# yweweler/single-speaker-tts

Measured on AMD Instinct MI355X. Metric: mel-frames/sec (end-to-end text->waveform incl. 60-iter Griffin-Lim, 64-utt LJ-Speech-shaped batch per GPU), higher is better.
Workload: dtype f32

## Files before the change

### single-speaker-tts_amd/csrc/gl_plan.h

```cpp
#pragma once
#include <cstddef>
#include <vector>

namespace tts {

constexpr int NFFT = 2048;
constexpr int MH = NFFT / 2;
constexpr int GL_NW = 8;
constexpr int EX_CPLX = 1088;
constexpr int CT_SWORDS = 16;
constexpr int GL_LDS_BUDGET = 160 * 1024;

struct GlItem { int b, t0, len, slot; };

struct GlStreamGeom { int wpad, halo, lag, S, acc_len; };
GlStreamGeom gl_stream_geom(int win, int hop);

int gl_stream_ring_frames(int win, int hop, int n_stage = 1);
size_t gl_stream_lds_bytes(int win, int hop, int ring_frames, int n_stage);

inline int gl_rw_edge_len(int n_fft, int win, int hop) { return n_fft + ((win + hop - 1) / hop - 1) * hop; }

void gl_build_wlane(const float* window, const float* rwss, int win, int hop, int T, float* out);

int gl_plan_items(const int* lens, int T, int B, int win, int hop, int n_workers, int n_stage, int force_runs, int force_run_len,
                  std::vector<GlItem>* items, int* slots_per_utt, int* workers_out = nullptr);

}
```

### single-speaker-tts_amd/csrc/gl_plan.hip

```cpp
#include "gl_plan.h"
#include <algorithm>
#include <cmath>
#include <utility>

namespace tts {

GlStreamGeom gl_stream_geom(int win, int hop) {
    GlStreamGeom g;
    g.wpad = (NFFT - win) >> 1;
    g.halo = (win + hop - 1) / hop - 1;
    g.lag = (g.halo + 1) * hop > 2 * (MH - g.wpad) ? g.halo : g.halo + 1;
    const int c_lo = g.wpad >> 7, c_hi = (g.wpad + win - 1) >> 7;
    g.S = 128 * (c_hi - c_lo + 1);
    g.acc_len = g.S - hop;
    return g;
}

static constexpr size_t GL_LDS_FIXED = (size_t)GL_NW * EX_CPLX * 2 * sizeof(float) + CT_SWORDS * sizeof(int);

int gl_stream_ring_frames(int win, int hop, int n_stage) {
    const GlStreamGeom g = gl_stream_geom(win, hop);
    if (g.acc_len < 0) return 0;
    const int budget = (GL_LDS_BUDGET - (int)GL_LDS_FIXED) / (int)sizeof(float) / n_stage - g.acc_len - 132;
    int need = 9 + g.lag + (g.S + hop - 1) / hop + 1;
    const int reach = (g.S + win + 2 * hop + hop - 1) / hop;
    need = std::max(need, std::max(reach, GL_NW));
    const int R = std::min(budget / hop, std::max(64, need));
    return R >= need ? R : 0;
}

size_t gl_stream_lds_bytes(int win, int hop, int ring_frames, int n_stage) {
    const GlStreamGeom g = gl_stream_geom(win, hop);
    return GL_LDS_FIXED + (size_t)(n_stage < 1 ? 1 : n_stage) * (size_t)((hop * ring_frames + g.acc_len + 128 + 3) & ~3) * sizeof(float);
}

void gl_build_wlane(const float* window, const float* rwss, int win, int hop, int T, float* out) {
    const GlStreamGeom g = gl_stream_geom(win, hop);
    const int t_ref = g.halo < T ? g.halo : T - 1;
    for (int c = 0; c < 16; ++c)
        for (int e = 0; e < 2; ++e)
            for (int lane = 0; lane < 64; ++lane) {
                const int nw = 2 * (lane + 64 * c) + e - g.wpad;
                const bool in = nw >= 0 && nw < win;
                const float w = in ? window[nw] * (0.5f / (float)MH) : 0.f;
                const float rw = in ? rwss[(size_t)t_ref * hop + g.wpad + nw] : 0.f;
                out[(0 * 64 + lane) * 32 + 2 * c + e] = w;
                out[(1 * 64 + lane) * 32 + 2 * c + e] = w * rw;
            }
}

namespace {
struct GlRun { int b, t0, len, ord = 0; };
struct GlCutCost { double interior, edge; };
GlCutCost gl_cut_cost(int halo, int lag, int n_stage) {
    const double c = (halo + lag) * n_stage / 4.0;
    return GlCutCost{c * (5.5 / 6.0), c * 0.5};
}
template <bool STORE>
bool gl_deal(const int* lens, int T, int B, int W, double M, const GlCutCost& cc, int min_len_all, std::vector<std::vector<GlRun>>& workers, double* makespan,
             double give_up = 1e300) {
    if (STORE) workers.assign((size_t)W, {});
    bool w_empty = true;
    int b = 0, t = 0, w = 0;
    double load = 0.0, worst = 0.0;
    while (b < B) {
        if (w >= W) return false;
        const int Tb = lens ? lens[b] : T;
        const int min_len = std::min(Tb, min_len_all);
        const int rest = Tb - t;
        const double left = t > 0 ? cc.interior : cc.edge;
        const double whole = rest + left + cc.edge;
        if (load + whole <= M + 1e-9) {
            if (STORE) workers[w].push_back(GlRun{b, t, rest});
            w_empty = false;
            load += whole;
            ++b; t = 0;
            continue;
        }
        int len = (int)std::floor(M - load - left - cc.interior + 1e-9);
        if (rest - len < min_len) len = rest - min_len;
        if (len >= min_len) {
            if (STORE) workers[w].push_back(GlRun{b, t, len});
            load += len + left + cc.interior;
            t += len;
        } else if (w_empty) {
            return false;
        }
        worst = std::max(worst, load);
        if (!STORE && worst >= give_up) return false;
        ++w; load = 0.0; w_empty = true;
    }
    worst = std::max(worst, load);
    if (makespan) *makespan = worst;
    return true;
}
}

int gl_plan_items(const int* lens, int T, int B, int win, int hop, int n_workers, int n_stage, int force_runs, int force_run_len,
                  std::vector<GlItem>* items, int* slots_per_utt, int* workers_out) {
    auto len_of = [&](int b) { return lens ? lens[b] : T; };
    long long total_frames = 0;
    int T_min = len_of(0), T_top = len_of(0);
    for (int b = 0; b < B; ++b) {
        total_frames += len_of(b);
        T_min = std::min(T_min, len_of(b));
        T_top = std::max(T_top, len_of(b));
    }
    if (lens && T_min == T_top) {
        lens = nullptr;
        T = T_top;
    }
    const GlStreamGeom g = gl_stream_geom(win, hop);
    n_stage = n_stage < 1 ? 1 : (n_stage > 3 ? 3 : n_stage);
    n_workers = n_workers < 1 ? 1 : n_workers;
    std::vector<std::vector<GlRun>> workers;
    int forced_len = 0;
    if (force_runs >= 1 && force_runs <= T_top) forced_len = ((T_top + force_runs - 1) / force_runs + GL_NW - 1) / GL_NW * GL_NW;
    if (force_run_len >= GL_NW) forced_len = force_run_len / GL_NW * GL_NW;
    if (forced_len > 0) {
        for (int t0 = 0; t0 < T_top; t0 += forced_len)
            for (int b = 0; b < B; ++b)
                if (t0 < len_of(b)) workers.push_back({GlRun{b, t0, std::min(forced_len, len_of(b) - t0)}});
    } else {
        const GlCutCost cc = gl_cut_cost(g.halo, g.lag, n_stage);
        const long long per_worker = total_frames / n_workers;
        const int min_len_all = (int)std::max<long long>(GL_NW / 2, std::min<long long>(GL_NW, per_worker));
        const int min_len = std::min(T_min, min_len_all);
        const double total = (double)total_frames + (double)B * 2 * cc.edge;
        double lo = std::max(total / n_workers, (double)min_len + 2 * cc.edge), best_t = 1e300;
        std::vector<std::vector<GlRun>> none;
        int best_step = -1;
        double best_M = 0.0;
        for (int step = 0; step < 400; ++step) {
            const double M = lo * (1.0 + 0.0025 * step);
            double t = 0.0;
            if (!gl_deal<false>(lens, T, B, n_workers, M, cc, min_len_all, none, &t, best_t - 1e-9)) continue;
            if (t < best_t - 1e-9) { best_t = t; best_M = M; best_step = step; }
        }
        if (lens && best_step > 0) {
            for (int sub = 1; sub < 16; ++sub) {
                const double M = lo * (1.0 + 0.0025 * (best_step - 1 + sub / 16.0));
                double t = 0.0;
                if (!gl_deal<false>(lens, T, B, n_workers, M, cc, min_len_all, none, &t, best_t - 1e-9)) continue;
                if (t < best_t - 1e-9) { best_t = t; best_M = M; }
            }
        }
        if (best_step >= 0) gl_deal<true>(lens, T, B, n_workers, best_M, cc, min_len_all, workers, nullptr);
        if (workers.empty()) {
            for (int b = 0; b < B; ++b) workers.push_back({GlRun{b, 0, len_of(b)}});
        }
    }
    std::vector<int> runs_of((size_t)B, 0);
    for (auto& w : workers) for (GlRun& r : w) r.ord = runs_of[r.b]++;
    int spu = 1;
    for (int b = 0; b < B; ++b) spu = std::max(spu, runs_of[b]);
    auto item_of = [&](const GlRun& r) {
        const int ord = r.ord;
        const int pad = ord == runs_of[r.b] - 1 ? spu - runs_of[r.b] : 0;
        return GlItem{r.b, r.t0, r.len, ord | (pad << 16)};
    };
    typedef std::pair<double, const GlRun*> Start;
    const auto earlier = [](const Start& a, const Start& b) { return a.first < b.first; };
    items->clear();
    size_t depth = 0;
    for (const auto& w : workers) depth = std::max(depth, w.size());
    if (lens) {
        std::vector<Start> rest;
        for (const auto& w : workers) {
            double before = 0.0;
            for (size_t d = 0; d < w.size(); ++d) {
                if (d == 0) items->push_back(item_of(w[d]));
                else rest.push_back({before, &w[d]});
                before += w[d].len + 11.0;
            }
        }
        std::stable_sort(rest.begin(), rest.end(), earlier);
        for (const auto& e : rest) items->push_back(item_of(*e.second));
        depth = 0;
    }
    for (size_t d = 0; d < depth; ++d) {
        std::vector<Start> level;
        for (const auto& w : workers) {
            if (w.size() <= d) continue;
            double before = 0.0;
            for (size_t q = 0; q < d; ++q) before += w[q].len;
            level.push_back({before, &w[d]});
// ... 15 lines not shown
```

### single-speaker-tts_amd/csrc/griffin_lim.hip

```cpp
#include "tts_common.h"
#include "griffin_lim.h"
#include "fft_wave.h"
#include <algorithm>
#include <cmath>
#include <cstdlib>

namespace tts {


__device__ __forceinline__ void lds_barrier() {
    asm volatile("s_waitcnt lgkmcnt(0)\n\ts_barrier" ::: "memory");
}

typedef __attribute__((address_space(3))) int gl_lds_int;
__device__ __forceinline__ int gl_flag_load(int* p) {
    return __hip_atomic_load((gl_lds_int*)p, __ATOMIC_RELAXED, __HIP_MEMORY_SCOPE_WORKGROUP);
}
__device__ __forceinline__ void gl_flag_store(int* p, int v) {
    __hip_atomic_store((gl_lds_int*)p, v, __ATOMIC_RELAXED, __HIP_MEMORY_SCOPE_WORKGROUP);
}

__device__ __forceinline__ void mirror_bins(const cf (&z)[16], cf (&m)[16], cf* ex, int lane, cf nyq) {
    cf* wr = ex + lane;
    const cf* rd = ex + (1024 - lane);
#pragma unroll
    for (int c = 0; c < 16; ++c) wr[64 * c] = z[c];
    if (lane == 0) ex[1024] = nyq;
    wave_lds_sync();
#pragma unroll
    for (int c = 0; c < 16; ++c) m[c] = rd[-64 * c];
    wave_lds_sync();
}

#define GL_BIN(lane, j) ((j) < 8 ? (lane) + 64 * (j) : MH - (lane) - 64 * ((j) - 8))
#define GL_ROW(LO, HI, j) ((j) < 8 ? (LO)[64 * (j)] : (HI)[-64 * ((j) - 8)])
#define GL_THREADS 512

__device__ __forceinline__ float gl_stream_load(const float* p) { return __builtin_nontemporal_load(p); }
__device__ __forceinline__ void gl_stream_store(cf* p, cf v) { __builtin_nontemporal_store(v, p); }
#define GL_STREAM_LOAD(ptr) gl_stream_load(ptr)
#define GL_STREAM_STORE(ptr, val) gl_stream_store((ptr), (val))
__device__ __forceinline__ cf gl_seed_phasor(unsigned long long seed, unsigned long long idx) {
    unsigned x = (unsigned)idx ^ ((unsigned)(idx >> 32) * 0x9E3779B9u) ^ (unsigned)seed ^ ((unsigned)(seed >> 32) * 0x85EBCA6Bu);
    x ^= x >> 16; x *= 0x7FEB352Du; x ^= x >> 15; x *= 0x846CA68Bu; x ^= x >> 16;
    const float u = (float)(x >> 8) * (1.0f / 16777216.0f);
    return cmk(__builtin_amdgcn_cosf(u), __builtin_amdgcn_sinf(u));
}
__device__ __forceinline__ unsigned gl_pack_phasor(cf x) {
    const float den = fmaxf(fabsf(x.x) + fabsf(x.y), 1.0e-30f);
    const float p = x.y * __builtin_amdgcn_rcpf(den);
    return (__float_as_uint(p) & ~1u) | (__float_as_uint(x.x) >> 31);
}
__device__ __forceinline__ cf gl_unpack_phasor(unsigned c, float mag) {
    const float p = __uint_as_float(c);
    const float q = 1.0f - fabsf(p);
    const float xs = __uint_as_float(__float_as_uint(q) | (c << 31));
    const float g = mag * __builtin_amdgcn_rsqf(fmaf(p, p, q * q));
    return cmk(xs, p) * g;
}

__device__ __forceinline__ cf gl_normalise(cf x, float mag) {
    const float xr = x.x + 1.0e-17f;
    const float s2 = fmaf(xr, xr, fmaf(x.y, x.y, 1.0e-38f));
    const float g = mag * __builtin_amdgcn_rsqf(s2);
    return cmk(xr, x.y) * g;
}
typedef unsigned gl_state_t;
__device__ __forceinline__ gl_state_t gl_state_encode(cf x) { return gl_pack_phasor(x); }
__device__ __forceinline__ cf gl_state_decode(gl_state_t s, float mag) { return gl_unpack_phasor(s, mag); }
size_t gl_state_bytes() { return sizeof(gl_state_t); }

#define GL_NO_ITEM 0x7FFFFFFEu
enum { CT_OLA = 0, CT_SNEXT = 1, CT_OLB = 2  };

template <int MODE, int WIN_CT, int HOP_CT, bool MSE, int NST = 1, bool SEEDED = false, bool MOM = false, bool RAG = false>
__global__ __launch_bounds__(GL_THREADS) void gl_stream_kernel(GlParams p) {
    static_assert(!SEEDED || MODE == 0, "the seeded start is an iteration's");
    static_assert(!MOM || (MODE == 0 && NST == 1), "momentum: one iteration per launch");
    static_assert(NST == 1 || (NST >= 2 && NST <= 3 && MODE == 0 && !MSE), "several iterations per launch: plain iterations only");
    extern __shared__ __attribute__((aligned(16))) unsigned char smem_raw[];
    const int win = WIN_CT ? WIN_CT : p.win;
    const int hop = HOP_CT ? HOP_CT : p.hop;
    const int ncol = (WIN_CT && HOP_CT) ? (WIN_CT + HOP_CT - 1) / (HOP_CT ? HOP_CT : 1) : p.ncol;
    const int halo = ncol - 1;
    const int wpad = (NFFT - win) >> 1;
    const int c_lo = wpad >> 7;
    const int c_hi = (wpad + win - 1) >> 7;
    constexpr int fz_lo_ = WIN_CT ? ((NFFT - WIN_CT) >> 1) >> 7 : 0;
    constexpr int fz_hi_ = WIN_CT ? (((NFFT - WIN_CT) >> 1) + WIN_CT - 1) >> 7 : 15;
    constexpr bool fz_ok_ = fz_lo_ <= 4 && fz_hi_ >= 11 && fz_hi_ <= 15;
    constexpr int FZ_LO = fz_ok_ ? fz_lo_ : 0, FZ_HI = fz_ok_ ? fz_hi_ : 15;
    const int n_sl = c_hi - c_lo + 1;
    const int S = 128 * n_sl;
    const int fs = 128 * c_lo;
    const int acc_len = S - hop;
    const int lag = (halo + 1) * hop > 2 * (MH - wpad) ? halo : halo + 1;
    const int R = p.ring_frames;
    const int ring_len = hop * R;
    const int ring_floats = (ring_len + acc_len + 128 + 3) & ~3;
    const int L = hop * (p.T - 1);
    int Tb_r = p.T;
    int L_r = L;
    const float* rw_head = nullptr;
    const float* rw_tail = nullptr;
#define GL_TB (RAG ? Tb_r : p.T)
#define GL_L (RAG ? L_r : L)
    cf* ex_all = reinterpret_cast<cf*>(smem_raw);
    int* ctrl = reinterpret_cast<int*>(ex_all + GL_NW * EX_CPLX);
    float* ringA = reinterpret_cast<float*>(ctrl + CT_SWORDS);

    const int tid = threadIdx.x;
    const int lane = tid & 63;
    const int wave = __builtin_amdgcn_readfirstlane(tid >> 6);
    cf* ex = ex_all + wave * EX_CPLX;

    if (tid == 0) ctrl[CT_SNEXT] = (int)atomicAdd(p.work_counter, 1u);
    if (tid == 0 && blockIdx.x == 0 && p.clear_counter) *p.clear_counter = 0u;
    cf twr[8];
#pragma unroll
    for (int j = 0; j < 8; ++j) twr[j] = reinterpret_cast<const cf*>(p.tw2048)[lane + 64 * j];
    FftTwReg tw;
#pragma unroll
    for (int k2 = 1; k2 < 16; ++k2) tw.a[k2 - 1] = reinterpret_cast<const cf*>(p.tables)[1024 + (k2 - 1) * 64 + lane];
#pragma unroll
    for (int d = 1; d < 4; ++d) tw.b[d - 1] = reinterpret_cast<const cf*>(p.tw1024)[16 * (lane & 15) * d];
    float wana[16][2], wsyn[16][2];
    {
        const float4* wa = reinterpret_cast<const float4*>(p.wlane + (0 * 64 + lane) * 32);
        const float4* ws = reinterpret_cast<const float4*>(p.wlane + (1 * 64 + lane) * 32);
#pragma unroll
        for (int q = 0; q < 8; ++q) {
            const float4 a4 = wa[q], s4 = ws[q];
            wana[2 * q][0] = a4.x; wana[2 * q][1] = a4.y; wana[2 * q + 1][0] = a4.z; wana[2 * q + 1][1] = a4.w;
            wsyn[2 * q][0] = s4.x; wsyn[2 * q][1] = s4.y; wsyn[2 * q + 1][0] = s4.z; wsyn[2 * q + 1][1] = s4.w;
        }
#pragma unroll
        for (int c = 0; c < 16; ++c)
            if (WIN_CT && (c < c_lo || c > c_hi)) { wana[c][0] = wana[c][1] = wsyn[c][0] = wsyn[c][1] = 0.f; }
#pragma unroll
        for (int c = 0; c < 16; ++c) wsyn[c][1] = -wsyn[c][1];
    }
    __syncthreads();
    int item = __builtin_amdgcn_readfirstlane(ctrl[CT_SNEXT]);

    auto decode_item = [&](int it, int& b, int& t0, int& len, int& slot, int& tb) {
        const int4 q = p.items[it];
        b = q.x; t0 = q.y; len = q.z; slot = q.w;
        if (RAG) tb = p.n_frames[q.x];
    };

    gl_state_t gc[16];
    float gs[16];
    gl_state_t nyq_c;
    float nyq_s;
    constexpr bool seeded = SEEDED;
#define GLS_LOAD_ROW(BASE_C, BASE_M, TF, TB)                                                    \
    {                                                                                           \
        int tf_ = (TF);                                                                         \
        tf_ = tf_ < 0 ? 0 : (tf_ >= (TB) ? (TB) - 1 : tf_);                                     \
        const gl_state_t* prow_ = (BASE_C) + (size_t)tf_ * p.FP;                                \
        const float* srow_ = (BASE_M) + (size_t)tf_ * p.FP;                                     \
        const gl_state_t* plo_ = prow_ + lane; const gl_state_t* phi_ = prow_ + (MH - lane);    \
        const float* slo_ = srow_ + lane; const float* shi_ = srow_ + (MH - lane);              \
        if (!seeded) {                                                                          \
            _Pragma("unroll") for (int j_ = 0; j_ < 16; ++j_) gc[j_] = GL_ROW(plo_, phi_, j_); \
            nyq_c = prow_[MH / 2];                                                              \
        }                                                                                       \
        _Pragma("unroll") for (int j_ = 0; j_ < 16; ++j_) gs[j_] = GL_STREAM_LOAD(j_ < 8 ? slo_ + 64 * j_ : shi_ - 64 * (j_ - 8)); \
        nyq_s = srow_[MH / 2];                                                                  \
    }
#define GLS_TOUCH_ROW()                                                                                              \
    asm volatile("" : "+v"(gc[0]), "+v"(gc[1]), "+v"(gc[2]), "+v"(gc[3]), "+v"(gc[4]), "+v"(gc[5]), "+v"(gc[6]),       \
                      "+v"(gc[7]), "+v"(gc[8]), "+v"(gc[9]), "+v"(gc[10]), "+v"(gc[11]), "+v"(gc[12]), "+v"(gc[13]), \
                      "+v"(gc[14]), "+v"(gc[15]), "+v"(nyq_c));                                                      \
    asm volatile("" : "+v"(gs[0]), "+v"(gs[1]), "+v"(gs[2]), "+v"(gs[3]), "+v"(gs[4]), "+v"(gs[5]), "+v"(gs[6]),       \
                      "+v"(gs[7]), "+v"(gs[8]), "+v"(gs[9]), "+v"(gs[10]), "+v"(gs[11]), "+v"(gs[12]), "+v"(gs[13]), \
                      "+v"(gs[14]), "+v"(gs[15]), "+v"(nyq_s));
    const gl_state_t* x_in = reinterpret_cast<const gl_state_t*>(p.phase_in);
    gl_state_t* x_out = reinterpret_cast<gl_state_t*>(p.phase_out);

#define GLS_URGENCY(NEXT_INDEX)                                                                    \
    {                                                                                              \
        const int d_ = __builtin_amdgcn_readfirstlane((NEXT_INDEX) - gl_flag_load(ctrl + CT_OLA)); \
        if (d_ <= 1) __builtin_amdgcn_s_setprio(3);                                                \
        else if (d_ <= 3) __builtin_amdgcn_s_setprio(2);                                           \
        else if (d_ <= 5) __builtin_amdgcn_s_setprio(1);                                           \
        else __builtin_amdgcn_s_setprio(0);                                                        \
    }

    auto split_pass = [&](cf (&gk)[16], cf mid, cf (&v)[16]) __attribute__((always_inline)) {
        cf* wr = ex + (MH - lane);
#pragma unroll
        for (int c = 0; c < 8; ++c) {
            cf xk = gk[c];
            cf xm = gk[8 + c];
            if (c == 0 && lane == 0) { xk.y = 0.f; xm.y = 0.f; }
            const cf e = cadd_conj(xk, xm);
            const cf o = cmul_conj(csub_conj(xk, xm), twr[c]);
            v[c] = cconj_add_pi(e, o);
            wr[-64 * c] = cadd_mi(e, o);
        }
        if (lane == 0) ex[MH / 2] = cscale(mid, 2.0f);
        wave_lds_sync();
#pragma unroll
        for (int j = 8; j < 16; ++j) v[j] = ex[lane + 64 * j];
        wave_lds_sync();
    };
    auto synth_window = [&](int t, cf (&v)[16]) __attribute__((always_inline)) {
        if (t >= halo && t + halo < GL_TB) {
#pragma unroll
            for (int c = 0; c < 16; ++c) v[c] = v[c] * cmk(wsyn[c][0], wsyn[c][1]);
        } else {
            const float* rwp = (RAG ? (t < halo ? rw_head : rw_tail) : p.rwss) + (size_t)t * hop + wpad;
#pragma unroll
            for (int c0 = 0; c0 < 16; c0 += 4) {
#pragma unroll
                for (int c = c0; c < c0 + 4; ++c) {
                    const int nw0 = 2 * (lane + 64 * c) - wpad;
                    const bool i0 = nw0 >= 0 && nw0 < win, i1 = nw0 + 1 >= 0 && nw0 + 1 < win;
                    const float r0 = rwp[i0 ? nw0 : 0], r1 = rwp[i1 ? nw0 + 1 : 0];
                    v[c] = cmk(i0 ? v[c].x * wana[c][0] * r0 : 0.f, i1 ? -v[c].y * wana[c][1] * r1 : 0.f);
                }
                asm volatile("" ::: "memory");
            }
        }
    };
    float pk = 0.f;
    auto overlap_add = [&](float* ring, int chain, int idx, int s, int t, int b, int run_t0, int run_len, const cf (&v)[16])
                           __attribute__((always_inline)) {
        float* const lds_f = reinterpret_cast<float*>(smem_raw);
        const int e_wr = (int)(ring - lds_f) + hop * s + 2 * lane;
        const int e_rd = e_wr + (s == 0 ? ring_len : 0);
        int wo[8], ro[8];
#pragma unroll
        for (int k = 0; k < 8; ++k) {
            wo[k] = e_wr + 256 * k;
            ro[k] = e_rd + 256 * k;
            if (2 * k < n_sl) asm volatile("" : "+v"(wo[k]), "+v"(ro[k]));
        }
        const int qb_edge = 128 * ((acc_len - 1) >> 7);
        unsigned keep0 = qb_edge + 2 * lane < acc_len ? ~0u : 0u, keep1 = qb_edge + 2 * lane + 1 < acc_len ? ~0u : 0u;
        asm volatile("" : "+v"(keep0), "+v"(keep1));
        while (gl_flag_load(ctrl + chain) < idx) __builtin_amdgcn_s_sleep(1);
        asm volatile("" ::: "memory");
        cf fin[16];
        {
            cf o[16];
#pragma unroll
            for (int c = 0; c < 16; ++c) {
                const int j = c - c_lo;
                o[c] = cmk(0.f, 0.f);
                if (j < 0 || j >= n_sl) continue;
                const int qb = 128 * j;
                const float* rp = lds_f + ro[j >> 1] + 128 * (j & 1);
                if (qb < acc_len) o[c] = cmk(rp[0], rp[1]);
            }
            asm volatile("" ::: "memory");
#pragma unroll
            for (int c = 0; c < 16; ++c) {
                const int j = c - c_lo;
                if (j < 0 || j >= n_sl) continue;
                const int qb = 128 * j;
                cf a = v[c];
                if (qb < acc_len) {
                    cf acc = o[c];
                    if (qb + 127 >= acc_len) {
                        acc.x = __uint_as_float(__float_as_uint(acc.x) & keep0);
                        acc.y = __uint_as_float(__float_as_uint(acc.y) & keep1);
                    }
                    a = cadd(acc, v[c]);
                }
                float* wp = lds_f + wo[j >> 1] + 128 * (j & 1);
                wp[0] = a.x;
                wp[1] = a.y;
                if (MODE == 1) fin[c] = a;
            }
        }
        asm volatile("" ::: "memory");
        if (lane == 0) gl_flag_store(ctrl + chain, idx + 1);
        if (MODE == 1) {
            asm volatile("" ::: "memory");
            const int q_fin = wpad - fs;
            const int y0 = t * hop + fs - MH;
            const bool emit = (t >= run_t0 || run_t0 == 0) && (t < run_t0 + run_len || run_t0 + run_len == GL_TB);
            float* wb = p.wav + (size_t)b * L;
#pragma unroll
            for (int c = 0; c < 16; ++c) {
                const int j = c - c_lo;
                if (j < 0 || j >= n_sl) continue;
                const int qb = 128 * j;
                if (qb + 127 >= q_fin && qb < q_fin + hop) {
                    const int q = qb + 2 * lane;
                    const int y = y0 + q;
                    const cf a = fin[c];
                    if (emit && q >= q_fin && q < q_fin + hop && y >= 0 && y < GL_L) { wb[y] = a.x; pk = fmaxf(pk, fabsf(a.x)); }
                    if (emit && q + 1 >= q_fin && q + 1 < q_fin + hop && y + 1 >= 0 && y + 1 < GL_L) { wb[y + 1] = a.y; pk = fmaxf(pk, fabsf(a.y)); }
                }
            }
        }
    };
    auto fft_input = [&](const float* ring, int idx, int sm, int tm, int y_base, cf (&v)[16]) __attribute__((always_inline)) {
        const int ylo = tm * hop + wpad - MH;
        const bool edge = ylo < 0 || ylo + win > GL_L;
        if (!edge && (hop * sm + S <= ring_len || R - sm > lag)) {
            const float* const lds_f = reinterpret_cast<const float*>(smem_raw);
            const int e_rd = (int)(ring - lds_f) + hop * sm + 2 * lane;
            int ro[8];
#pragma unroll
            for (int k = 0; k < 8; ++k) {
                ro[k] = e_rd + 256 * k;
                if (2 * k < n_sl) asm("" : "+v"(ro[k]));
            }
#pragma unroll
            for (int c = 0; c < 16; ++c) {
                const int j = c - c_lo;
                if (j < 0 || j >= n_sl) { v[c] = cmk(0.f, 0.f); continue; }
                const float* sf = lds_f + ro[j >> 1] + 128 * (j & 1);
                v[c] = cmk(wana[c][0], wana[c][1]) * cmk(sf[0], sf[1]);
            }
        } else {
            const int lap0 = (idx - lag) / R;
            const int ub = y_base + lap0 * ring_len;
#pragma unroll
            for (int c = 0; c < 16; ++c) {
                float x[2] = {0.f, 0.f};
#pragma unroll
                for (int e = 0; e < 2; ++e) {
                    const int f = 2 * (lane + 64 * c) + e;
                    const int nw = f - wpad;
                    if (nw >= 0 && nw < win) {
                        int y = ylo + nw;
                        y = y < 0 ? -y : y;
                        y = y >= GL_L ? 2 * (GL_L - 1) - y : y;
                        int off = y - ub, lap = lap0;
                        if (off >= ring_len) { off -= ring_len; ++lap; }
                        else if (off < 0) { off += ring_len; --lap; }
                        const int pos = (off < acc_len && lap * R > idx) ? ring_len + off : off;
                        x[e] = wana[c][e] * ring[pos];
                    }
                }
                v[c] = cmk(x[0], x[1]);
            }
        }
    };
    auto merge_pass = [&](const cf (&v)[16], auto&& sink) __attribute__((always_inline)) -> cf {
#pragma unroll
        for (int j = 8; j < 16; ++j) ex[lane + 64 * j] = v[j];
        if (lane == 0) ex[MH] = v[0];
        wave_lds_sync();
        cf zm[8];
        const cf* rd = ex + (MH - lane);
#pragma unroll
        for (int c = 0; c < 8; ++c) zm[c] = rd[-64 * c];
#pragma unroll
        for (int c = 0; c < 8; ++c) {
            const cf e = cadd_conj(v[c], zm[c]);
            const cf o = cmul(csub_conj(v[c], zm[c]), twr[c]);
            sink(c, cadd_mi(e, o));
            sink(8 + c, cconj_add_pi(e, o));
        }
        wave_lds_sync();
        return cscale(cconj(v[8]), 2.0f);
    };

    const int lead = NST * halo;
    bool have_row = false;
    while (item < p.n_items) {
        int b, run_t0, run_len, slot;
        decode_item(item, b, run_t0, run_len, slot, Tb_r);
        if (RAG) {
            L_r = hop * (Tb_r - 1);
            const int cut = NFFT + L_r - p.rw_E;
            rw_head = p.rw_edge + (size_t)b * 2 * p.rw_E;
            rw_tail = rw_head + p.rw_E - (cut > 0 ? cut : 0);
        }
        const float* magb = p.mag + (size_t)b * p.T * p.FP;
        const gl_state_t* phb = x_in + (size_t)b * p.T * p.FP;
        const int n_idx = run_len + NST * (halo + lag);
        const bool late = n_idx >= 4 * GL_NW;
        const int i_res = n_idx - 3 * GL_NW;
        unsigned next_item_reg = GL_NO_ITEM;
        if (tid == 0 && !late) next_item_reg = atomicAdd(p.work_counter, 1u);
        if (!have_row) GLS_LOAD_ROW(phb, magb, run_t0 - lead + wave, GL_TB)
        have_row = false;
        for (int q = tid; q < acc_len + 128; q += GL_THREADS) {
#pragma unroll
            for (int k = 0; k < NST; ++k) ringA[k * ring_floats + ring_len + q] = 0.f;
        }
        if (tid == 0) { ctrl[CT_OLA] = 0; ctrl[CT_OLB] = 0; ctrl[CT_OLB + 1] = 0; ctrl[CT_SNEXT] = (int)next_item_reg; }
        __syncthreads();
        int next_item = __builtin_amdgcn_readfirstlane(ctrl[CT_SNEXT]);
        int nb = b, nt0 = 0, nlen = 0, nslot = 0, nTb = p.T;
        if (!late && next_item < p.n_items) decode_item(next_item, nb, nt0, nlen, nslot, nTb);

        const int y_base_a = (run_t0 - lead) * hop - MH + fs;
        float mse_acc = 0.f;
        pk = 0.f;
        int s = wave % R;
        GLS_TOUCH_ROW()
        for (int i = wave; i < n_idx; i += GL_NW) {
            const int t = run_t0 - lead + i;
            const bool valid = t >= 0 && t < GL_TB;
            unsigned drawn = 0;
            if (late && i == i_res && lane == 0) drawn = atomicAdd(p.work_counter, 1u);
            if (late && i + GL_NW >= n_idx) {
                int nv;
                while ((nv = gl_flag_load(ctrl + CT_SNEXT)) == (int)GL_NO_ITEM) __builtin_amdgcn_s_sleep(1);
                next_item = __builtin_amdgcn_readfirstlane(nv);
                if (next_item < p.n_items) decode_item(next_item, nb, nt0, nlen, nslot, nTb);
            }
            GLS_URGENCY(i)
            cf v[16];
            if (valid) {
                cf gk[16];
                if (seeded) {
                    const unsigned long long row0 = (unsigned long long)b * p.F * p.T + (unsigned long long)t;
#pragma unroll
                    for (int j = 0; j < 16; ++j) {
                        const cf e = gl_seed_phasor(p.seed, row0 + (unsigned long long)GL_BIN(lane, j) * p.T);
                        gk[j] = cmk(gs[j] * e.x, gs[j] * e.y);
                    }
                    const cf en = gl_seed_phasor(p.seed, row0 + (unsigned long long)(MH / 2) * p.T);
                    split_pass(gk, cmk(nyq_s * en.x, nyq_s * en.y), v);
                } else {
#pragma unroll
                    for (int j = 0; j < 16; ++j) gk[j] = gl_state_decode(gc[j], gs[j]);
                    split_pass(gk, gl_state_decode(nyq_c, nyq_s), v);
                }
            } else {
#pragma unroll
                for (int j = 0; j < 16; ++j) asm volatile("v_mov_b64 %0, 0" : "=v"(v[j]));
            }
            GLS_URGENCY(i)
#define GLS_NEXT_ROW()                                                                                                   \
            if (i + GL_NW < n_idx) {                                                                                     \
                GLS_LOAD_ROW(phb, magb, t + GL_NW, GL_TB)                                                                \
            } else if (next_item < p.n_items) {                                                                          \
                GLS_LOAD_ROW(x_in + (size_t)nb * p.T * p.FP, p.mag + (size_t)nb * p.T * p.FP, nt0 - lead + wave, (RAG ? nTb : p.T)) \
                have_row = true;                                                                                         \
            }
            if (NST == 1) {
                GLS_NEXT_ROW()
            }
            if (valid) {
                fft1024(v, ex, tw, lane);
                synth_window(t, v);
            }
            if (late && i == i_res && lane == 0) gl_flag_store(ctrl + CT_SNEXT, (int)drawn);
            overlap_add(ringA, CT_OLA, i, s, t, b, run_t0, run_len, v);
            if (NST == 1) {
                GLS_TOUCH_ROW()
            }
            GLS_URGENCY(i + GL_NW)

            int sk = s, ik = i, tk = t;
            float* ring_k = ringA;
            int yb_k = y_base_a;
#pragma nounroll
            for (int k = 1; k < NST; ++k) {
                const int i_prev = ik, s_prev = sk;
                const float* ring_prev = ring_k;
                const int yb_prev = yb_k;
                ik -= halo + lag;
                tk -= lag;
                sk -= halo + lag;
                sk += sk < 0 ? R : 0;
                ring_k += ring_floats;
                yb_k += halo * hop;
                const bool valid_k = ik >= 0 && tk >= 0 && tk < GL_TB;
                {
                    const int tq = tk < 0 ? 0 : (tk >= GL_TB ? GL_TB - 1 : tk);
                    const float* mrow_ = magb + (size_t)tq * p.FP;
                    const float* mlo_ = mrow_ + lane; const float* mhi_ = mrow_ + (MH - lane);
#pragma unroll
                    for (int j = 0; j < 16; ++j) gs[j] = GL_ROW(mlo_, mhi_, j);
                    nyq_s = mrow_[MH / 2];
                }
                if (valid_k) {
                    int sm = s_prev - lag;
                    sm += sm < 0 ? R : 0;
                    fft_input(ring_prev, i_prev, sm, tk, yb_prev, v);
                    fft1024<FZ_LO, FZ_HI>(v, ex, tw, lane);
                    cf gk[16];
                    const cf xmid = merge_pass(v, [&](int c, cf x) { gk[c] = gl_normalise(x, gs[c]); });
                    split_pass(gk, gl_normalise(xmid, nyq_s), v);
                } else {
#pragma unroll
                    for (int j = 0; j < 16; ++j) asm volatile("v_mov_b64 %0, 0" : "=v"(v[j]));
                }
                if (k + 1 == NST) {
                    GLS_NEXT_ROW()
                }
                if (ik >= 0) {
                    if (valid_k) {
                        fft1024(v, ex, tw, lane);
                        synth_window(tk, v);
                    }
                    overlap_add(ring_k, CT_OLB + k - 1, ik, sk, tk, b, run_t0, run_len, v);
                }
            }
            if (NST > 1) GLS_TOUCH_ROW()
            const int jj = ik, sb = sk;
            if (MODE == 0 && jj >= halo + lag && jj < halo + lag + run_len) {
                const int tm = tk - lag;
                int sm = sb - lag;
                sm += sm < 0 ? R : 0;
                const float* mrow = magb + (size_t)tm * p.FP;
                float mg[16];
                if (MSE) {
#pragma unroll
                    for (int c = 0; c < 16; ++c) mg[c] = fabsf(GL_STREAM_LOAD(c < 8 ? mrow + lane + 64 * c : mrow + (MH - lane) - 64 * (c - 8)));
                }
                cf cp[16], cp_mid = cmk(0.f, 0.f);
                cf* const crow = MOM ? reinterpret_cast<cf*>(p.mom_c) + ((size_t)b * p.T + tm) * p.FP : nullptr;
                cf* const clo = MOM ? crow + lane : nullptr;
                cf* const chi = MOM ? crow + (MH - lane) : nullptr;
                const bool mom_prev = MOM && !p.mom_first;
                if (MOM) {
#pragma unroll
                    for (int c = 0; c < 16; ++c) cp[c] = cmk(0.f, 0.f);
                    if (mom_prev) {
#pragma unroll
                        for (int c = 0; c < 16; ++c) cp[c] = __builtin_nontemporal_load(c < 8 ? clo + 64 * c : chi - 64 * (c - 8));
                        cp_mid = crow[MH / 2];
                    }
                }
                auto mom_t = [&](cf x, cf prev) __attribute__((always_inline)) -> cf {
                    return mom_prev ? cadd(x, cscale(csub(x, prev), p.mom_alpha)) : x;
                };
                fft_input(ring_k, jj, sm, tm, yb_k, v);
                fft1024<FZ_LO, FZ_HI>(v, ex, tw, lane);
                GLS_URGENCY(i + GL_NW)
                if (MOM && MSE) mse_acc = 0.f;
                gl_state_t* orow = x_out + ((size_t)b * p.T + tm) * p.FP;
                gl_state_t* olo = orow + lane;
                gl_state_t* ohi = orow + (MH - lane);
                const cf xmid = merge_pass(v, [&](int c, cf x) {
                    if (MOM) {
                        GL_STREAM_STORE(c < 8 ? clo + 64 * c : chi - 64 * (c - 8), x);
                        __builtin_nontemporal_store(gl_state_encode(mom_t(x, cp[c])), c < 8 ? olo + 64 * c : ohi - 64 * (c - 8));
                    } else
                    __builtin_nontemporal_store(gl_state_encode(x), c < 8 ? olo + 64 * c : ohi - 64 * (c - 8));
                    if (MSE) {
                        const float d = mg[c] - (float)MH * sqrtf(fmaf(x.x, x.x, x.y * x.y));
                        mse_acc += d * d;
                    }
                });
                if (lane == 0) {
                    if (MOM) crow[MH / 2] = xmid;
                    __builtin_nontemporal_store(gl_state_encode(MOM ? mom_t(xmid, cp_mid) : xmid), orow + MH / 2);
                    if (MSE) {
                        const float d = fabsf(mrow[MH / 2]) - (float)MH * sqrtf(fmaf(xmid.x, xmid.x, xmid.y * xmid.y));
                        mse_acc += d * d;
                    }
                }
                if (MOM && MSE) {
                    float r = mse_acc;
#pragma unroll
                    for (int o = 32; o > 0; o >>= 1) r += __shfl_xor(r, o);
                    if (lane == 0) p.mse_partial[(size_t)b * p.T + tm] = r;
                }
            }
            s += GL_NW;
            s -= s >= R ? R : 0;
        }
        __builtin_amdgcn_s_setprio(0);
        if ((MODE == 0 && MSE && !MOM) || (MODE == 1 && p.peak_partial)) {
            float r = MODE == 0 ? mse_acc : pk;
#pragma unroll
            for (int o = 32; o > 0; o >>= 1) r = MODE == 0 ? r + __shfl_xor(r, o) : fmaxf(r, __shfl_xor(r, o));
            __syncthreads();
            float* red = reinterpret_cast<float*>(ex_all);
            if (lane == 0) red[wave] = r;
            __syncthreads();
            if (tid == 0) {
                float a = 0.f;
                for (int w = 0; w < GL_NW; ++w) a = MODE == 0 ? a + red[w] : fmaxf(a, red[w]);
                float* part = (MODE == 0 ? p.mse_partial : p.peak_partial) + (size_t)b * p.slots_per_utt + (slot & 0xffff);
                part[0] = a;
                for (int q = 1; q <= (slot >> 16); ++q) part[q] = 0.f;
            }
        }
        __syncthreads();
        item = next_item;
    }
#undef GLS_LOAD_ROW
#undef GL_TB
#undef GL_L
#undef GLS_NEXT_ROW
#undef GLS_TOUCH_ROW
#undef GLS_URGENCY
}


bool gl_stream_instantiated(int win, int hop) { return (win == 1102 && hop == 275) || (win == 800 && hop == 200); }

typedef void (*GlStreamKernel)(GlParams);
template <int W, int H, bool RAG>
static GlStreamKernel gl_stream_form_wh(bool final_istft, bool mse, int n_stage, bool seeded, bool mom) {
    if (final_istft) return (mse || n_stage != 1 || seeded || mom) ? nullptr : &gl_stream_kernel<1, W, H, false, 1, false, false, RAG>;
    if (mom) {
        if (n_stage != 1 || (mse && seeded)) return nullptr;
        if (mse) return &gl_stream_kernel<0, W, H, true, 1, false, true, RAG>;
        return seeded ? &gl_stream_kernel<0, W, H, false, 1, true, true, RAG> : &gl_stream_kernel<0, W, H, false, 1, false, true, RAG>;
    }
    if (mse)
        return n_stage != 1 ? nullptr : seeded ? &gl_stream_kernel<0, W, H, true, 1, true, false, RAG> : &gl_stream_kernel<0, W, H, true, 1, false, false, RAG>;
    switch (n_stage) {
        case 1: return seeded ? &gl_stream_kernel<0, W, H, false, 1, true, false, RAG> : &gl_stream_kernel<0, W, H, false, 1, false, false, RAG>;
        case 2: return seeded ? &gl_stream_kernel<0, W, H, false, 2, true, false, RAG> : &gl_stream_kernel<0, W, H, false, 2, false, false, RAG>;
        case 3: return seeded ? &gl_stream_kernel<0, W, H, false, 3, true, false, RAG> : &gl_stream_kernel<0, W, H, false, 3, false, false, RAG>;
    }
    return nullptr;
}
static GlStreamKernel gl_stream_form(int win, int hop, bool rag, bool final_istft, bool mse, int n_stage, bool seeded, bool mom) {
    if (win == 1102 && hop == 275)
        return rag ? gl_stream_form_wh<1102, 275, true>(final_istft, mse, n_stage, seeded, mom) : gl_stream_form_wh<1102, 275, false>(final_istft, mse, n_stage, seeded, mom);
    if (win == 800 && hop == 200)
        return rag ? gl_stream_form_wh<800, 200, true>(final_istft, mse, n_stage, seeded, mom) : gl_stream_form_wh<800, 200, false>(final_istft, mse, n_stage, seeded, mom);
    return nullptr;
}

hipError_t launch_gl_stream(hipStream_t s, const GlParams& p_in, int n_cus, int final_istft, int n_stage) {
    GlParams p = p_in;
    p.n_stage = n_stage;
    if (n_stage < 1 || n_stage > 3) return hipErrorInvalidValue;
    p.ring_frames = gl_stream_ring_frames(p.win, p.hop, n_stage);
    if (p.ring_frames < GL_NW) return hipErrorInvalidValue;
    if (p.n_frames && (!p.rw_edge || p.rw_E != gl_rw_edge_len(NFFT, p.win, p.hop))) return hipErrorInvalidValue;
    const GlStreamKernel kernel = gl_stream_form(p.win, p.hop, p.n_frames != nullptr, final_istft != 0, p.mse_partial != nullptr, n_stage,
                                                 p.seeded != 0, p.mom_c && !final_istft);
    if (!kernel) return hipErrorInvalidValue;
    const int nwg = p.n_workers > 0 && p.n_workers < n_cus ? p.n_workers : (p.n_items < n_cus ? p.n_items : n_cus);
    hipLaunchKernelGGL(kernel, dim3(nwg), dim3(GL_THREADS), gl_stream_lds_bytes(p.win, p.hop, p.ring_frames, n_stage), s, p);
    return hipGetLastError();
}

static hipError_t gl_stream_configure() {
    for (int wh = 0; wh < 2; ++wh)
        for (int rag = 0; rag < 2; ++rag)
            for (int i = 0; i < 16 * 3; ++i) {
                const bool final_istft = i & 1, mse = i & 2, seeded = i & 4, mom = i & 8;
                const GlStreamKernel kernel = gl_stream_form(wh ? 800 : 1102, wh ? 200 : 275, rag, final_istft, mse, 1 + i / 16, seeded, mom);
                if (!kernel) continue;
                const hipError_t e = hipFuncSetAttribute(reinterpret_cast<const void*>(kernel), hipFuncAttributeMaxDynamicSharedMemorySize, GL_LDS_BUDGET);
                if (e != hipSuccess) return e;
            }
    return hipSuccess;
}

__global__ __launch_bounds__(GL_THREADS) void stft_kernel(const float* __restrict__ wav, int n, int Tf,
                                                          const float* __restrict__ window, int win, int hop,
                                                          const cf* __restrict__ tw1024, const cf* __restrict__ tw2048,
                                                          cf* __restrict__ out, int FP) {
    extern __shared__ __attribute__((aligned(16))) unsigned char smem_raw[];
    cf* ex_all = reinterpret_cast<cf*>(smem_raw);
    cf* twR = ex_all + GL_NW * EX_CPLX;
    cf* twA = twR + 1024;
    float* wtab = reinterpret_cast<float*>(twA + 15 * 64);
    const int tid = threadIdx.x, lane = tid & 63, wave = tid >> 6;
    cf* ex = ex_all + wave * EX_CPLX;
    for (int i = tid; i < win; i += GL_THREADS) wtab[i] = window[i];
    for (int i = tid; i < 1024; i += GL_THREADS) twR[i] = tw2048[i];
    for (int i = tid; i < 15 * 64; i += GL_THREADS) twA[i] = tw1024[(i & 63) * ((i >> 6) + 1)];
    FftTw tw;
#pragma unroll
    for (int d = 1; d < 4; ++d) tw.b[d - 1] = tw1024[16 * (lane & 15) * d];
    tw.a = twA + lane;
    __syncthreads();
    const int b = blockIdx.y;
    const int t = blockIdx.x * GL_NW + wave;
    if (t >= Tf) return;
    const float* y = wav + (size_t)b * n;
    const int wpad = (NFFT - win) >> 1;
    const int ylo = t * hop + wpad - MH;
    cf v[16];
#pragma unroll
    for (int j = 0; j < 16; ++j) {
        const int nn = 2 * (lane + 64 * j);
        float x[2] = {0.f, 0.f};
#pragma unroll
        for (int e = 0; e < 2; ++e) {
            const int nw = nn + e - wpad;
            if (nw >= 0 && nw < win) {
                int yi = ylo + nw;
                yi = yi < 0 ? -yi : yi;
                yi = yi >= n ? 2 * (n - 1) - yi : yi;
                x[e] = wtab[nw] * y[yi];
            }
        }
        v[j] = cmk(x[0], x[1]);
    }
    fft1024(v, ex, tw, lane);
#pragma unroll
    for (int c = 0; c < 16; ++c) ex[lane + 64 * c] = v[c];
    wave_lds_sync();
    cf* orow = out + ((size_t)b * Tf + t) * FP;
#pragma unroll
    for (int c = 0; c < 16; ++c) {
        const int k = lane + 64 * c;
        const cf zk = v[c];
        const cf zr = ex[(MH - k) & (MH - 1)];
        const cf e = cscale(cadd_conj(zk, zr), 0.5f);
        const cf o = cmul(cscale(csub_conj(zk, zr), 0.5f), twR[k]);
        orow[k] = cadd_mi(e, o);
    }
    if (lane == 0) orow[MH] = cmk(v[0].x - v[0].y, 0.f);
    if (lane < FP - MH - 1) orow[MH + 1 + lane] = cmk(0.f, 0.f);
}

static hipError_t stft_configure() {
    return hipFuncSetAttribute(reinterpret_cast<const void*>(&stft_kernel), hipFuncAttributeMaxDynamicSharedMemorySize, GL_LDS_BUDGET);
}
hipError_t gl_configure() {
    const hipError_t e = gl_stream_configure();
    return e != hipSuccess ? e : stft_configure();
}

hipError_t launch_stft(hipStream_t s, const float* wav, int B, int n, int Tf, const float* window, int win, int hop,
                       const float2* tw1024, const float2* tw2048, float2* out, int FP) {
    const size_t lds = (size_t)(GL_NW * EX_CPLX + 1024 + 15 * 64) * sizeof(cf) + (size_t)((win + 3) & ~3) * sizeof(float);
    dim3 grid((Tf + GL_NW - 1) / GL_NW, B);
    hipLaunchKernelGGL(stft_kernel, grid, dim3(GL_THREADS), lds, s, wav, n, Tf, window, win, hop,
                       reinterpret_cast<const cf*>(tw1024), reinterpret_cast<const cf*>(tw2048), reinterpret_cast<cf*>(out), FP);
    return hipGetLastError();
}

__global__ void cplx_tf_to_ft_kernel(const cf* in, float* out, int F, int T, int FP, int mode, float power) {
    __shared__ cf tile[32][33];
    const int b = blockIdx.z;
    const int f0 = blockIdx.y * 32, t0 = blockIdx.x * 32;
    const int tx = threadIdx.x, ty = threadIdx.y;
    for (int i = ty; i < 32; i += 8) {
        const int t = t0 + i, f = f0 + tx;
        tile[i][tx] = (t < T && f < F) ? in[((size_t)b * T + t) * FP + f] : cmk(0.f, 0.f);
    }
    __syncthreads();
    for (int i = ty; i < 32; i += 8) {
        const int f = f0 + i, t = t0 + tx;
// ... 219 lines not shown
```

Measured before the change: 4.384 million.

## Deinterleave LDS ring buffer into even/odd halves per 128-sample block

Changes the physical layout of the overlap-add ring in LDS so each 128-sample block stores even samples then odd samples. Lane accesses become unit-stride 32-bit loads instead of stride-2 pairs, meant to cut LDS bank conflicts in the overlap-add and FFT-input paths. Ring allocation is rounded up to 128 floats, and ring-frame selection now decrements to stay within the LDS budget. Odd-hop bases need separate address paths, and the wrap case needs per-element selection, which adds complexity and extra register use.

```diff
diff --git a/single-speaker-tts_amd/csrc/gl_plan.h b/single-speaker-tts_amd/csrc/gl_plan.h
--- a/single-speaker-tts_amd/csrc/gl_plan.h
+++ b/single-speaker-tts_amd/csrc/gl_plan.h
@@ -10,6 +10,14 @@
 constexpr int EX_CPLX = 1088;
 constexpr int CT_SWORDS = 16;
 constexpr int GL_LDS_BUDGET = 160 * 1024;
+
+#if defined(__HIPCC__) || defined(__CUDACC__)
+#define GL_HD __host__ __device__
+#else
+#define GL_HD
+#endif
+GL_HD constexpr int gl_ring_phys(int q) { return (q & ~127) + ((q & 1) << 6) + ((q & 127) >> 1); }
+GL_HD constexpr int gl_ring_alloc_floats(int hop, int ring_frames, int acc_len) { return (hop * ring_frames + acc_len + 128 + 127) & ~127; }
 
 struct GlItem { int b, t0, len, slot; };
 
diff --git a/single-speaker-tts_amd/csrc/gl_plan.hip b/single-speaker-tts_amd/csrc/gl_plan.hip
--- a/single-speaker-tts_amd/csrc/gl_plan.hip
+++ b/single-speaker-tts_amd/csrc/gl_plan.hip
@@ -25,13 +25,14 @@
     int need = 9 + g.lag + (g.S + hop - 1) / hop + 1;
     const int reach = (g.S + win + 2 * hop + hop - 1) / hop;
     need = std::max(need, std::max(reach, GL_NW));
-    const int R = std::min(budget / hop, std::max(64, need));
+    int R = std::min(budget / hop, std::max(64, need));
+    while (R >= need && gl_stream_lds_bytes(win, hop, R, n_stage) > (size_t)GL_LDS_BUDGET) --R;
     return R >= need ? R : 0;
 }
 
 size_t gl_stream_lds_bytes(int win, int hop, int ring_frames, int n_stage) {
     const GlStreamGeom g = gl_stream_geom(win, hop);
-    return GL_LDS_FIXED + (size_t)(n_stage < 1 ? 1 : n_stage) * (size_t)((hop * ring_frames + g.acc_len + 128 + 3) & ~3) * sizeof(float);
+    return GL_LDS_FIXED + (size_t)(n_stage < 1 ? 1 : n_stage) * (size_t)gl_ring_alloc_floats(hop, ring_frames, g.acc_len) * sizeof(float);
 }
 
 void gl_build_wlane(const float* window, const float* rwss, int win, int hop, int T, float* out) {
diff --git a/single-speaker-tts_amd/csrc/griffin_lim.hip b/single-speaker-tts_amd/csrc/griffin_lim.hip
--- a/single-speaker-tts_amd/csrc/griffin_lim.hip
+++ b/single-speaker-tts_amd/csrc/griffin_lim.hip
@@ -13,6 +13,8 @@
 }
 
 typedef __attribute__((address_space(3))) int gl_lds_int;
+typedef __attribute__((address_space(3))) float gl_lds_float;
+typedef __attribute__((address_space(3))) unsigned char gl_lds_char;
 __device__ __forceinline__ int gl_flag_load(int* p) {
     return __hip_atomic_load((gl_lds_int*)p, __ATOMIC_RELAXED, __HIP_MEMORY_SCOPE_WORKGROUP);
 }
@@ -97,7 +99,7 @@
     const int lag = (halo + 1) * hop > 2 * (MH - wpad) ? halo : halo + 1;
     const int R = p.ring_frames;
     const int ring_len = hop * R;
-    const int ring_floats = (ring_len + acc_len + 128 + 3) & ~3;
+    const int ring_floats = gl_ring_alloc_floats(hop, R, acc_len);
     const int L = hop * (p.T - 1);
     int Tb_r = p.T;
     int L_r = L;
@@ -225,19 +227,32 @@
             }
         }
     };
+    constexpr bool HOP_ODD = HOP_CT == 0 || (HOP_CT & 1);
+    const int lds0 = (int)(unsigned long long)(gl_lds_char*)smem_raw;
+    auto ring_addr = [&](int r0, int base, int k) __attribute__((always_inline)) -> int {
+        const int bk = base + k;
+        const int w = 2 * (bk & 127) + 4 * lane;
+        return lds0 + 4 * (r0 + (bk & ~127)) + 256 * (bk & 1) + (w & 0x1FC) + (w & 0x100);
+    };
+#define GL_LDS_F(ADDR) (*(gl_lds_float*)(unsigned long long)(unsigned)(ADDR))
     float pk = 0.f;
     auto overlap_add = [&](float* ring, int chain, int idx, int s, int t, int b, int run_t0, int run_len, const cf (&v)[16])
                            __attribute__((always_inline)) {
-        float* const lds_f = reinterpret_cast<float*>(smem_raw);
-        const int e_wr = (int)(ring - lds_f) + hop * s + 2 * lane;
-        const int e_rd = e_wr + (s == 0 ? ring_len : 0);
-        int wo[8], ro[8];
-#pragma unroll
-        for (int k = 0; k < 8; ++k) {
-            wo[k] = e_wr + 256 * k;
-            ro[k] = e_rd + 256 * k;
-            if (2 * k < n_sl) asm volatile("" : "+v"(wo[k]), "+v"(ro[k]));
-        }
+        const int r0 = (int)(ring - reinterpret_cast<float*>(smem_raw));
+        const int base_wr = hop * s;
+        const bool wr_odd = HOP_ODD && (base_wr & 1);
+        bool rd_odd = wr_odd;
+        int wx = ring_addr(r0, base_wr, 0), wy = wx + 256;
+        if (wr_odd) wy = ring_addr(r0, base_wr, 1);
+        int rx = wx, ry = wy;
+        if (s == 0) {
+            int fold = ring_len;
+            asm volatile("" : "+s"(fold));
+            rd_odd = HOP_ODD && (fold & 1);
+            rx = ring_addr(r0, fold, 0);
+            ry = rd_odd ? ring_addr(r0, fold, 1) : rx + 256;
+        }
+        asm volatile("" : "+v"(wx), "+v"(wy), "+v"(rx), "+v"(ry));
         const int qb_edge = 128 * ((acc_len - 1) >> 7);
         unsigned keep0 = qb_edge + 2 * lane < acc_len ? ~0u : 0u, keep1 = qb_edge + 2 * lane + 1 < acc_len ? ~0u : 0u;
         asm volatile("" : "+v"(keep0), "+v"(keep1));
@@ -247,33 +262,64 @@
         {
             cf o[16];
 #pragma unroll
-            for (int c = 0; c < 16; ++c) {
-                const int j = c - c_lo;
-                o[c] = cmk(0.f, 0.f);
-                if (j < 0 || j >= n_sl) continue;
-                const int qb = 128 * j;
-                const float* rp = lds_f + ro[j >> 1] + 128 * (j & 1);
-                if (qb < acc_len) o[c] = cmk(rp[0], rp[1]);
-            }
-            asm volatile("" ::: "memory");
-#pragma unroll
-            for (int c = 0; c < 16; ++c) {
-                const int j = c - c_lo;
-                if (j < 0 || j >= n_sl) continue;
-                const int qb = 128 * j;
-                cf a = v[c];
-                if (qb < acc_len) {
-                    cf acc = o[c];
-                    if (qb + 127 >= acc_len) {
-                        acc.x = __uint_as_float(__float_as_uint(acc.x) & keep0);
-                        acc.y = __uint_as_float(__float_as_uint(acc.y) & keep1);
-                    }
-                    a = cadd(acc, v[c]);
-                }
-                float* wp = lds_f + wo[j >> 1] + 128 * (j & 1);
-                wp[0] = a.x;
-                wp[1] = a.y;
-                if (MODE == 1) fin[c] = a;
+            for (int c = 0; c < 16; ++c) o[c] = cmk(0.f, 0.f);
+            auto masked = [&](int qb, cf acc) __attribute__((always_inline)) -> cf {
+                if (qb + 127 >= acc_len) {
+                    acc.x = __uint_as_float(__float_as_uint(acc.x) & keep0);
+                    acc.y = __uint_as_float(__float_as_uint(acc.y) & keep1);
+                }
+                return acc;
+            };
+            if (!rd_odd && !wr_odd) {
+                int bx = rx, cx = wx;
+                asm volatile("" : "+v"(bx), "+v"(cx));
+#pragma unroll
+                for (int c = 0; c < 16; ++c) {
+                    const int j = c - c_lo;
+                    if (j < 0 || j >= n_sl) continue;
+                    if (128 * j < acc_len) o[c] = cmk(GL_LDS_F(bx + 512 * j), GL_LDS_F(bx + 512 * j + 256));
+                }
+                asm volatile("" ::: "memory");
+#pragma unroll
+                for (int c = 0; c < 16; ++c) {
+                    const int j = c - c_lo;
+                    if (j < 0 || j >= n_sl) continue;
+                    o[c] = 128 * j < acc_len ? cadd(masked(128 * j, o[c]), v[c]) : v[c];
+                    GL_LDS_F(cx + 512 * j) = o[c].x;
+                    GL_LDS_F(cx + 512 * j + 256) = o[c].y;
+                }
+                asm volatile("" ::: "memory");
+            } else {
+                int bx = rx, by = ry, cx = wx, cy = wy;
+                asm volatile("" : "+v"(bx), "+v"(by), "+v"(cx), "+v"(cy));
+#pragma unroll
+                for (int c = 0; c < 16; ++c) {
+                    const int j = c - c_lo;
+                    if (j < 0 || j >= n_sl) continue;
+                    if (128 * j < acc_len) o[c] = cmk(GL_LDS_F(bx + 512 * j), GL_LDS_F(by + 512 * j));
+                }
+                asm volatile("" ::: "memory");
+#pragma unroll
+                for (int c = 0; c < 16; ++c) {
+                    const int j = c - c_lo;
+                    if (j < 0 || j >= n_sl) continue;
+                    const cf acc = masked(128 * j, o[c]);
+                    o[c] = 128 * j < acc_len ? cmk(acc.x + v[c].x, acc.y + v[c].y) : v[c];
+                }
+#pragma unroll
+                for (int c = c_lo; c < c_lo + n_sl; c += 2) {
+                    const int j = c - c_lo;
+                    const bool two = j + 1 < n_sl;
+                    GL_LDS_F(cx + 512 * j) = o[c & 15].x;
+                    if (two) GL_LDS_F(cx + 512 * j + 512) = o[(c + 1) & 15].x;
+                    GL_LDS_F(cy + 512 * j) = o[c & 15].y;
+                    if (two) GL_LDS_F(cy + 512 * j + 512) = o[(c + 1) & 15].y;
+                }
+                asm volatile("" ::: "memory");
+            }
+            if (MODE == 1) {
+#pragma unroll
+                for (int c = 0; c < 16; ++c) fin[c] = o[c];
             }
         }
         asm volatile("" ::: "memory");
@@ -302,21 +348,40 @@
     auto fft_input = [&](const float* ring, int idx, int sm, int tm, int y_base, cf (&v)[16]) __attribute__((always_inline)) {
         const int ylo = tm * hop + wpad - MH;
         const bool edge = ylo < 0 || ylo + win > GL_L;
-        if (!edge && (hop * sm + S <= ring_len || R - sm > lag)) {
-            const float* const lds_f = reinterpret_cast<const float*>(smem_raw);
-            const int e_rd = (int)(ring - lds_f) + hop * sm + 2 * lane;
-            int ro[8];
-#pragma unroll
-            for (int k = 0; k < 8; ++k) {
-                ro[k] = e_rd + 256 * k;
-                if (2 * k < n_sl) asm("" : "+v"(ro[k]));
-            }
+        const int r0 = (int)(ring - reinterpret_cast<const float*>(smem_raw));
+        const int base = hop * sm;
+        const bool odd = HOP_ODD && (base & 1);
+        if (!edge && (base + S <= ring_len || R - sm > lag)) {
+            int rx = ring_addr(r0, base, 0);
+            if (!odd) {
+                asm volatile("" : "+v"(rx));
+#pragma unroll
+                for (int c = 0; c < 16; ++c) {
+                    const int j = c - c_lo;
+                    if (j < 0 || j >= n_sl) { v[c] = cmk(0.f, 0.f); continue; }
+                    v[c] = cmk(wana[c][0], wana[c][1]) * cmk(GL_LDS_F(rx + 512 * j), GL_LDS_F(rx + 512 * j + 256));
+                }
+            } else {
+                int ry = ring_addr(r0, base, 1);
+                asm volatile("" : "+v"(rx), "+v"(ry));
+#pragma unroll
+                for (int c = 0; c < 16; ++c) {
+                    const int j = c - c_lo;
+                    if (j < 0 || j >= n_sl) { v[c] = cmk(0.f, 0.f); continue; }
+                    v[c] = cmk(wana[c][0] * GL_LDS_F(rx + 512 * j), wana[c][1] * GL_LDS_F(ry + 512 * j));
+                }
+            }
+        } else if (!edge) {
+            int a0 = ring_addr(r0, base, 0), a1 = ring_addr(r0, base, 1);
+            int b0 = ring_addr(r0, base - ring_len, 0), b1 = ring_addr(r0, base - ring_len, 1);
+            int left = ring_len - base - 2 * lane;
+            asm volatile("" : "+v"(a0), "+v"(a1), "+v"(b0), "+v"(b1), "+v"(left));
 #pragma unroll
             for (int c = 0; c < 16; ++c) {
                 const int j = c - c_lo;
                 if (j < 0 || j >= n_sl) { v[c] = cmk(0.f, 0.f); continue; }
-                const float* sf = lds_f + ro[j >> 1] + 128 * (j & 1);
-                v[c] = cmk(wana[c][0], wana[c][1]) * cmk(sf[0], sf[1]);
+                const int px = (128 * j < left ? a0 : b0) + 512 * j, py = (128 * j + 1 < left ? a1 : b1) + 512 * j;
+                v[c] = cmk(wana[c][0] * GL_LDS_F(px), wana[c][1] * GL_LDS_F(py));
             }
         } else {
             const int lap0 = (idx - lag) / R;
@@ -336,7 +401,7 @@
                         if (off >= ring_len) { off -= ring_len; ++lap; }
                         else if (off < 0) { off += ring_len; --lap; }
                         const int pos = (off < acc_len && lap * R > idx) ? ring_len + off : off;
-                        x[e] = wana[c][e] * ring[pos];
+                        x[e] = wana[c][e] * ring[gl_ring_phys(pos)];
                     }
                 }
                 v[c] = cmk(x[0], x[1]);
@@ -385,7 +450,7 @@
         have_row = false;
         for (int q = tid; q < acc_len + 128; q += GL_THREADS) {
 #pragma unroll
-            for (int k = 0; k < NST; ++k) ringA[k * ring_floats + ring_len + q] = 0.f;
+            for (int k = 0; k < NST; ++k) ringA[k * ring_floats + gl_ring_phys(ring_len + q)] = 0.f;
         }
         if (tid == 0) { ctrl[CT_OLA] = 0; ctrl[CT_OLB] = 0; ctrl[CT_OLB + 1] = 0; ctrl[CT_SNEXT] = (int)next_item_reg; }
         __syncthreads();
@@ -585,6 +650,7 @@
         item = next_item;
     }
 #undef GLS_LOAD_ROW
+#undef GL_LDS_F
 #undef GL_TB
 #undef GL_L
 #undef GLS_NEXT_ROW
```

Result: no change. 4.422 million (median of 6 runs) (+0.9%).
